# szpajder/dumphfdl

Measured on AMD Instinct MI355X. Metric: wideband I/Q Msamples/s (cf32 ingest -> decoded HFDL PDUs) at fixed channel count, higher is better.
Workload: dtype f32

## Files before the change

### dumphfdl_amd/csrc/frontend.h

```cpp
#pragma once
#include <hip/hip_runtime.h>
#include <deque>
#include <memory>
#include <vector>
#include "../../include/hfdl_gpu.h"
#include "hip_handles.h"
#include "kernels.h"
#include "planner.h"
#include "demod.h"
#include "spectrum.h"
#include "export_ring.h"

namespace hfdl {

int select_device(int device);
long env_long(const char *name, long lo, long hi, long otherwise);
inline int ilog2(int x) { int l = 0; while ((1 << l) < x) l++; return l; }
inline size_t sample_bytes(int fmt) { return fmt == SFMT_CS16 ? 4 : fmt == SFMT_CU8 ? 2 : 8; }
bool is_library_pinned(const void *p, size_t bytes);

struct LabConfig {
	int fold_tile = -1;
	int fold_slices = 0;
	int cu_split = 0;
// ... 62 lines not shown
	PinnedBuf<float> host;
	std::vector<Event> ev;
	std::vector<hfdl_gpu_spectrum_row> info;
	uint64_t open = 0;
	uint64_t open_first = 0;
	uint32_t open_blocks = 0;
	uint64_t oldest() const { const uint64_t kept = (uint64_t)rows - (open_blocks ? 1 : 0); return open > kept ? open - kept : 0; }
	void close()
	{
		info[open % (uint64_t)rows] = hfdl_gpu_spectrum_row{ open, open_first, open_blocks, 0 };
		open++;
		open_blocks = 0;
	}
};

struct SpectrumMonitor {
	int bins = 0;
	uint32_t flags = 0;
	DevBuf acc;
	DevBuf peak;
	PinnedBuf<float> host;
	Event ev;
	hipEvent_t last = nullptr;
	hipEvent_t newest() const { return last ? last : ev.e; }
	uint64_t fresh = 0;
	std::vector<uint64_t> blocks, first;
	std::unique_ptr<SpectrumHistory> hist;
};

struct ChannelExport {
	int nsel = 0, format = 0;
	float scale = 1.f;
	ExportRing ring;
	DevBuf channels;
	DevBuf samples, counts, power, clipped;
	size_t chunk = 1;
	PinnedBuf<char> host;
	std::vector<Event> ev;
	std::vector<uint64_t> last_of;
	hipEvent_t newest = nullptr;
};

}

struct hfdl_gpu_frontend {
	int device = 0;
	hfdl::Stream stream;
	hfdl::Stream stream_b;
	hfdl::Stream stream_d;
	hfdl::Stream stream_c;
	hfdl::Stream stream_f;
	bool cu_partitioned = false;
	bool own_decode_stream() const { return stream_d.owned; }
	bool fft_own_stream() const { return stream_f.owned; }
	static constexpr int MAX_HALF = hfdl::FOLD_MAX_BLOCKS;
	static constexpr int MAX_STAGE = HFDL_GPU_PREFETCH_MAX + 1;
	static_assert(MAX_HALF == hfdl::PLAN_MAX_HALF && MAX_STAGE == hfdl::PLAN_MAX_STAGE && HFDL_GPU_FOLD_BATCH_MAX == MAX_HALF, "include/hfdl_gpu.h, kernels.h and planner.h name the same limits");

	std::deque<hfdl::DevBuf> mem;
	template <typename T> hipError_t alloc(T *&view, size_t count)
	{
		mem.emplace_back();
		const hipError_t e = mem.back().alloc(sizeof(T) * count);
		view = mem.back().as<T>();
		return e;
	}
	hfdl::HostFftPlan fft;
	hfdl::Demod demod;
	int4 *d_rx = nullptr, *d_grp = nullptr;
	float2 *d_hist[2] = { nullptr, nullptr }, *d_work = nullptr, *d_spec = nullptr, *d_taps = nullptr, *d_partial = nullptr;
	float2 *d_tw_m = nullptr;
	int n_stage = 0;
	std::unique_ptr<hfdl::DevBuf> d_stage[MAX_STAGE];
	size_t stage_cap[MAX_STAGE] = {};
	float2 *d_chan_all = nullptr;
	int *d_cnt_all = nullptr;
	hfdl::ChanConst *d_cc = nullptr;
	int2 *d_win = nullptr;
	hfdl::NcoState *d_nco = nullptr;
	hfdl::NcoState *d_nco_snap = nullptr;
	float2 *d_ph = nullptr, *d_ph_cont = nullptr;
	std::unique_ptr<hfdl::SpectrumMonitor> mon;
	std::unique_ptr<hfdl::ChannelExport> exp;

	hfdl::DoneEvent dm[2][MAX_HALF];
	hfdl::DoneEvent chan[2];
	hfdl::DoneEvent fft_done;
	hfdl::DoneEvent spec[2];
	hfdl::Event ev_demod[2];
	hfdl::Event ev_stage_ready[MAX_STAGE];
	hfdl::Event ev_stage_free[MAX_STAGE];
	hfdl::LaunchTimers timers;
	int settle_events();

	uint64_t host_blocks = 0;
	uint64_t host_pushed = 0;
	const void *pf_ptr[MAX_STAGE] = {};
	int pf_fmt[MAX_STAGE] = {};
	hipEvent_t input_event(uint64_t host_block) const
	{
		const uint64_t newest = host_blocks - 1, span = (uint64_t)n_stage - 1;
		return ev_stage_ready[(newest - host_block <= span ? host_block : newest - span) % (uint64_t)n_stage];
	}
	int32_t sample_rate = 0, decimation = 0;
	float tbw = 0;
	hfdl::Plan plan{};
	hfdl::Geometry geo{};
	std::vector<int32_t> freqs;
	int nrx = 1;
	std::vector<int32_t> rx_center;
	std::vector<int32_t> rx_of;
	std::vector<hfdl::RxSpan> rx_span;
	std::vector<int4> rx_host;
	int slot_of(int c) const { return hfdl::receiver_slot(rx_span[(size_t)rx_of[(size_t)c]], c); }
	std::vector<hfdl::ChanConst> cc;
	int batch = 1;
	int fold_nb = 1;
	int half_blocks = 1;
	int half_first = 1, half_target = 1;
	int cur_half = 0, batch_fill = 0;
	int last_slot = 0;
	int last_index = 0;
	float2 *chan_slot(int slot) const { return d_chan_all + (size_t)slot * (size_t)geo.nch * (size_t)geo.outs; }
	int *cnt_slot(int slot) const { return d_cnt_all + (size_t)slot * (size_t)geo.nch; }
	int last_set = 0;
	float2 *spec_slot(int set, int i) const { return d_spec + ((size_t)set * (size_t)half_blocks + (size_t)i) * spec_stride(); }
	size_t spec_stride() const { return (size_t)nrx * (size_t)geo.n; }
	float2 *ph_slot(int set, int i) const { return d_ph + ((size_t)set * (size_t)half_blocks + (size_t)i) * ph_stride(); }
	hfdl::NcoState *snap_slot(int set, int i) const { return d_nco_snap + ((size_t)set * (size_t)half_blocks + (size_t)i) * (size_t)geo.nch; }
	size_t partial_stride() const { return (size_t)geo.nch * (size_t)geo.slices * (size_t)geo.m; }
	size_t ph_stride() const { return (size_t)geo.nch * (size_t)geo.outs; }
	double prune_tol = 0.0;
	int fold_rows_max = 0;
	bool fold_bound = false;
	uint64_t blocks = 0;
	hfdl::FftOutLayout tap_layout;
	int pending_demod_buf = -1;
	int pending_demod_nblk = 0;
	bool frames_wait_on_a = false;
	int demod_buf = -1;
	int prev_demod_buf = -1;
// ... 4 lines not shown
```

### dumphfdl_amd/csrc/frontend_create.cpp

```cpp
#include <atomic>
#include <cmath>
#include <complex>
#include <cstring>
#include <thread>
#include "frontend.h"

using namespace hfdl;

extern "C" int hfdl_gpu_device_count(void)
{
	int n = 0;
	if (hipGetDeviceCount(&n) != hipSuccess) return 0;
	return n;
}

int hfdl::select_device(int device)
{
	int n = 0;
	if (hipGetDeviceCount(&n) != hipSuccess || n <= 0)
		return fail(HFDL_GPU_ENODEV, "no HIP device visible: the HFDL front end has no CPU fallback");
	if (device < 0 || device >= n) return fail(HFDL_GPU_EINVAL, "device %d out of range (%d visible)", device, n);
	HIP_TRY(hipSetDevice(device));
	hipDeviceProp_t prop;
	HIP_TRY(hipGetDeviceProperties(&prop, device));
// ... 126 lines not shown
{
	if (!out || !centerfreqs || !freqs || !nch_per_rx) return fail(HFDL_GPU_EINVAL, "bad arguments: null pointer");
	*out = nullptr;
	if (nrx < 1 || nrx > HFDL_GPU_RECEIVERS_MAX) return fail(HFDL_GPU_EINVAL, "bad arguments: %d receivers (1 .. %d)", nrx, HFDL_GPU_RECEIVERS_MAX);
	for (int r = 0; r < nrx; r++)
		if (nch_per_rx[r] <= 0) return fail(HFDL_GPU_EINVAL, "bad arguments: receiver %d has %d channels", r, nch_per_rx[r]);
	if (sample_rate < 5400) return fail(HFDL_GPU_EINVAL, "sample rate must be >= 5400 (src/main.c:638-641)");
	for (int r = 0, c = 0; r < nrx; r++)
		for (int i = 0; i < nch_per_rx[r]; i++, c++)
			if (std::abs((int64_t)centerfreqs[r] - freqs[c]) >= sample_rate / 2)
				return nrx == 1 ? fail(HFDL_GPU_EINVAL, "channel %d Hz outside +-fs/2 of centre %d", freqs[c], centerfreqs[r])
				                : fail(HFDL_GPU_EINVAL, "channel %d (%d Hz) outside +-fs/2 of the centre %d of its receiver %d", c, freqs[c], centerfreqs[r], r);
	return 0;
}

extern "C" int hfdl_gpu_frontend_create(hfdl_gpu_frontend **out, int device, int32_t sample_rate, int32_t centerfreq,
		const int32_t *freqs, int32_t nch)
{
	if (!out || !freqs || nch <= 0) return fail(HFDL_GPU_EINVAL, "bad arguments");
	return hfdl_gpu_frontend_create_multi(out, device, sample_rate, 1, &centerfreq, freqs, &nch);
}

static int create_streams(hfdl_gpu_frontend *fe, const LabConfig &lab)
{
	CuPartition part = plan_cu_partition((int)fe->freqs.size(), Demod::workgroup_lds(), fe->fold_bound);
	if (!lab.cu_partition || lab.cu_split) part.on = false;
	if (part.on) {
		const hipError_t ea = fe->stream.create_on_cus(part.mask_fold), eb = fe->stream_b.create_on_cus(part.mask_demod);
		if (ea != hipSuccess || eb != hipSuccess) {
			fe->stream.reset(); fe->stream_b.reset();
			(void)hipGetLastError();
			(void)fail(0, "CU-masked streams refused (%s): the demodulators share the fold's CUs", hipGetErrorString(ea != hipSuccess ? ea : eb));
			part.on = false;
		}
	}
	fe->cu_partitioned = part.on;
	if (part.on) {
	} else if (lab.cu_split) {
		uint32_t mask_a[8] = {}, mask_b[8] = {};
		for (int i = 0; i < 256; i++)
			((((i >> 3) + i) % lab.cu_split) == 0 ? mask_b : mask_a)[i >> 5] |= 1u << (i & 31);
		CREATE_TRY(fe->stream.create_on_cus(mask_a));
		CREATE_TRY(fe->stream_b.create_on_cus(mask_b));
	} else {
		CREATE_TRY(fe->stream.create());
		CREATE_TRY(fe->stream_b.create());
	}
	if (lab.decode_stream) CREATE_TRY(fe->stream_d.create());
	else fe->stream_d.alias(fe->stream_b);
	fe->demod.separate_decode = fe->own_decode_stream();
	if (lab.fft_stream < 0 ? part.on : lab.fft_stream != 0) {
		if (part.on) CREATE_TRY(fe->stream_f.create_on_cus(part.mask_fold));
		else CREATE_TRY(fe->stream_f.create());
	} else fe->stream_f.alias(fe->stream);
	CREATE_TRY(fe->stream_c.create());
	return 0;
}

static int create_frontend(hfdl_gpu_frontend *fe, int32_t nrx, const int32_t *nch_per_rx)
{
	const int nch = (int)fe->freqs.size();
	const LabConfig lab = read_lab_config();
	if (!plan_block(fe->plan, fe->tbw, fe->decimation, 0.f)) return fail(HFDL_GPU_EINVAL, "fastddc planning failed");
	const Plan &pl = fe->plan;
	Geometry &g = fe->geo;
	g.n = pl.n; g.m = pl.m; g.pre = pl.pre; g.post = pl.post; g.scrap = pl.scrap; g.post_input_size = pl.post_input_size;
	g.overlap = pl.overlap; g.input_size = pl.input_size; g.outs = (pl.post_input_size + pl.post - 1) / pl.post + 1;
	g.nch = nch;
	g.tap_layout = (pl.m % 16) == 0 && (pl.pre % 8) == 0 ? TAPL_OCTET : TAPL_PLAIN;
	g.nch_pad = plan_receiver_slots(nch_per_rx, nrx, tap_layout_group(g.tap_layout), fe->rx_span);
	for (const RxSpan &r : fe->rx_span) fe->rx_host.push_back(make_int4(r.slot0, r.slots, r.chan0, r.nch));
	g.nrx = nrx;
	g.spec_rx_stride = pl.n;
	g.rx_host = fe->rx_host.data();
	g.tap_chan_stride = pl.m; g.tap_row_stride = (int64_t)g.nch_pad * pl.m;
	g.fold_tile = lab.fold_tile;
	fe->tap_layout.kind = g.tap_layout;
	fe->tap_layout.row_log = ilog2(pl.m); fe->tap_layout.row_stride = g.tap_row_stride;
	fe->prune_tol = g.tap_layout == TAPL_OCTET && nrx == 1 ? env_double("HFDL_GPU_FOLD_PRUNE", 1e-12, 1e-3, 0.0) : 0.0;
	fe->fold_bound = lab.fold_bound < 0 ? nch >= 128 : lab.fold_bound != 0;
	const float resamp_rate = (float)(1800 * 3) / ((float)fe->sample_rate / (float)fe->decimation);
	BatchOverrides ov;
	ov.demod_batch = (int)env_long("HFDL_GPU_DEMOD_BATCH", 1, 8, 0);
	ov.fold_batch = (int)env_long("HFDL_GPU_FOLD_BATCH", 1, hfdl_gpu_frontend::MAX_HALF, 0);
	ov.pruned = fe->prune_tol > 0;
	ov.fold_slices = lab.fold_slices;
	ov.no_ramp = !lab.fold_ramp;
	const BatchPlan bp = plan_batches(nch, nrx, pl.n, pl.input_size, fe->sample_rate, pl.pre, fe->fold_bound,
			[&](int want) { return Demod::fit_batch(g.outs, resamp_rate, want); }, ov);
	g.slices = bp.slices;
	g.rows_per_slice = pl.pre / g.slices;
	if (pl.m > 8192 || pl.m < 16) return fail(HFDL_GPU_ERANGE, "inverse FFT size %d unsupported", pl.m);

	if (int rc = create_streams(fe, lab)) return rc;
	for (int i = 0; i < 2; i++) {
		CREATE_TRY(fe->spec[i].own.create(EV_NO_TIMING));
		CREATE_TRY(fe->chan[i].own.create(EV_NO_TIMING));
		CREATE_TRY(fe->ev_demod[i].create(EV_NO_TIMING));
		for (DoneEvent &d : fe->dm[i]) CREATE_TRY(d.own.create(EV_NO_TIMING));
	}
	CREATE_TRY(fe->fft_done.own.create(EV_NO_TIMING));
	if (int rc = fe->fft.build(pl.n)) return rc;
	const size_t n = (size_t)pl.n;
	const size_t K = (size_t)nrx;
	for (int i = 0; i < 2; i++) {
		CREATE_TRY(fe->alloc(fe->d_hist[i], (size_t)pl.overlap * K));
		CREATE_TRY(hipMemsetAsync(fe->d_hist[i], 0, sizeof(float2) * (size_t)pl.overlap * K, fe->stream));
	}
	CREATE_TRY(fe->alloc(fe->d_work, n * K));
	CREATE_TRY(fe->alloc(fe->d_rx, K));
	CREATE_TRY(hipMemcpy(fe->d_rx, fe->rx_host.data(), sizeof(int4) * K, hipMemcpyHostToDevice));
	g.rx_tab = fe->d_rx;
	if (g.tap_layout == TAPL_OCTET) {
		static_assert(sizeof(FoldGroup) == sizeof(int4), "a FoldGroup entry is what the fold kernels load as an int4");
		const std::vector<FoldGroup> t = fold_group_tables(fe->rx_span, g.nch_pad / 8, FOLD_GROUP_MAX);
		CREATE_TRY(fe->alloc(fe->d_grp, t.size()));
		CREATE_TRY(hipMemcpy(fe->d_grp, t.data(), sizeof(int4) * t.size(), hipMemcpyHostToDevice));
		g.grp_tab = fe->d_grp;
	}
	CREATE_TRY(fe->alloc(fe->d_taps, n * (size_t)g.nch_pad));
	CREATE_TRY(fe->alloc(fe->d_nco, (size_t)nch));
	CREATE_TRY(hipMemsetAsync(fe->d_nco, 0, sizeof(NcoState) * (size_t)nch, fe->stream));
	CREATE_TRY(fe->alloc(fe->d_ph_cont, (size_t)nch));
	CREATE_TRY(fe->alloc(fe->d_cc, (size_t)nch));
	fe->mem.emplace_back();
	if (int rc = upload_twiddles(pl.m, fe->mem.back())) return rc;
	fe->d_tw_m = fe->mem.back().as<float2>();
	if (prepare_ifft_nco(pl.m) != hipSuccess)
		return fail(HFDL_GPU_EHIP, "inverse FFT of %d points: LDS attribute refused: %s", pl.m, hipGetErrorString(hipGetLastError()));
	if (int rc = build_taps(fe)) return rc;
	if (fe->prune_tol > 0 && g.tap_layout == TAPL_OCTET)
		if (int rc = build_fold_windows(fe)) return rc;
	CREATE_TRY(hipMemcpy(fe->d_cc, fe->cc.data(), sizeof(ChanConst) * (size_t)nch, hipMemcpyHostToDevice));
	fe->fold_nb = bp.fold_nb;
	if (int rc = fe->demod.init(nch, g.outs, resamp_rate, fe->freqs.data(), fe->stream, bp.batch_want)) return rc;
	fe->batch = fe->demod.batch;
	fe->half_blocks = bp.half_blocks;
	fe->half_first = fe->half_target = bp.half_first;
	fe->n_stage = bp.n_stage;
	for (int i = 0; i < fe->n_stage; i++) {
		CREATE_TRY(fe->ev_stage_ready[i].create(EV_NO_TIMING));
		CREATE_TRY(fe->ev_stage_free[i].create(EV_NO_TIMING));
	}
	const size_t hb = (size_t)fe->half_blocks;
	CREATE_TRY(fe->alloc(fe->d_spec, fe->spec_stride() * 2 * hb));
	CREATE_TRY(fe->alloc(fe->d_partial, fe->partial_stride() * hb));
	CREATE_TRY(fe->alloc(fe->d_ph, fe->ph_stride() * 2 * hb));
	CREATE_TRY(fe->alloc(fe->d_nco_snap, (size_t)nch * 2 * hb));
	CREATE_TRY(fe->alloc(fe->d_chan_all, 2 * hb * (size_t)nch * g.outs));
	CREATE_TRY(fe->alloc(fe->d_cnt_all, 2 * hb * (size_t)nch));
	CREATE_TRY(hipMemsetAsync(fe->d_cnt_all, 0, sizeof(int) * 2 * hb * (size_t)nch, fe->stream));
	CREATE_TRY(hipStreamSynchronize(fe->stream));
	return 0;
}
// ... 31 lines not shown
```

### dumphfdl_amd/csrc/frontend_query.cpp

```cpp
#include <algorithm>
#include <cstdarg>
#include <cstdio>
#include <cstring>
#include <mutex>
#include "frontend.h"

using namespace hfdl;

static thread_local char g_err[512] = "";

int hfdl::fail(int code, const char *fmt, ...)
{
	va_list ap;
	va_start(ap, fmt);
	vsnprintf(g_err, sizeof(g_err), fmt, ap);
	va_end(ap);
	return code;
}

int hfdl::fail_hip(hipError_t e, bool alloc, const char *expr, const char *file, int line)
{
	return fail(alloc && e == hipErrorOutOfMemory ? HFDL_GPU_ENOMEM : HFDL_GPU_EHIP, "%s: %s (%s:%d)", expr, hipGetErrorString(e), file, line);
}

// ... 33 lines not shown
	memset(g, 0, sizeof(*g));
	fill_block_geometry(p, g);
	g->decimation = decimation;
	g->transition_bw = transition_bw;
	return 0;
}

extern "C" int hfdl_gpu_frontend_channel_receiver(const hfdl_gpu_frontend *fe, int32_t channel, int32_t *rx, int32_t *centerfreq)
{
	if (!fe || !rx || !centerfreq) return fail(HFDL_GPU_EINVAL, "null argument");
	if (channel < 0 || channel >= fe->geo.nch) return fail(HFDL_GPU_EINVAL, "channel %d out of range (%d channels)", channel, fe->geo.nch);
	*rx = fe->rx_of[(size_t)channel];
	*centerfreq = fe->rx_center[(size_t)*rx];
	return 0;
}


static std::mutex g_pinned_lock;
static std::vector<std::pair<const char *, size_t>> g_pinned;

bool hfdl::is_library_pinned(const void *p, size_t bytes)
{
	std::lock_guard<std::mutex> lk(g_pinned_lock);
	for (auto &r : g_pinned)
		if ((const char *)p >= r.first && (const char *)p + bytes <= r.first + r.second) return true;
	return false;
}

extern "C" int hfdl_gpu_host_alloc(void **ptr, size_t bytes)
{
	if (!ptr || !bytes) return fail(HFDL_GPU_EINVAL, "bad arguments");
	HIP_TRY(hipHostMalloc(ptr, bytes, hipHostMallocDefault));
	std::lock_guard<std::mutex> lk(g_pinned_lock);
	g_pinned.emplace_back((const char *)*ptr, bytes);
	return 0;
}

extern "C" void hfdl_gpu_host_free(void *ptr)
{
	if (!ptr) return;
	{
		std::lock_guard<std::mutex> lk(g_pinned_lock);
		for (size_t i = 0; i < g_pinned.size(); i++)
			if (g_pinned[i].first == (const char *)ptr) { g_pinned.erase(g_pinned.begin() + (long)i); break; }
	}
	(void)hipHostFree(ptr);
}


extern "C" int hfdl_gpu_frontend_input_done(hfdl_gpu_frontend *fe)
{
	if (!fe) return fail(HFDL_GPU_EINVAL, "null argument");
	HIP_TRY(hipSetDevice(fe->device));
	HIP_TRY(hipStreamSynchronize(fe->stream_c));
	return 0;
}

static int check_host_block(const hfdl_gpu_frontend *fe, uint64_t host_block)
{
	if (!fe) return fail(HFDL_GPU_EINVAL, "null argument");
	if (host_block >= fe->host_blocks) return fail(HFDL_GPU_EINVAL, "host block %llu has not been pushed (%llu so far)", (unsigned long long)host_block, (unsigned long long)fe->host_blocks);
	HIP_TRY(hipSetDevice(fe->device));
	return 0;
}

extern "C" int hfdl_gpu_frontend_input_done_upto(hfdl_gpu_frontend *fe, uint64_t host_block)
{
	if (int rc = check_host_block(fe, host_block)) return rc;
	HIP_TRY(hipEventSynchronize(fe->input_event(host_block)));
	return 0;
}

extern "C" int hfdl_gpu_frontend_input_copied(hfdl_gpu_frontend *fe, uint64_t host_block)
{
	if (int rc = check_host_block(fe, host_block)) return rc;
	const hipError_t e = hipEventQuery(fe->input_event(host_block));
	if (e == hipSuccess) return 1;
	if (e == hipErrorNotReady) { (void)hipGetLastError(); return 0; }
	return fail(HFDL_GPU_EHIP, "hipEventQuery: %s", hipGetErrorString(e));
}


static int sync_to_read(hfdl_gpu_frontend *fe, bool args_ok = true)
{
	if (!fe || !args_ok) return fail(HFDL_GPU_EINVAL, "null argument");
	return hfdl_gpu_frontend_sync(fe);
}

extern "C" int hfdl_gpu_frontend_reset_timers(hfdl_gpu_frontend *fe, int enable)
{
	if (int rc = sync_to_read(fe)) return rc;
	return fe->timers.reset(enable != 0);
}

static int stage_totals(hfdl_gpu_frontend *fe, Stage s, double *ms, int64_t *launches, int64_t *blocks)
{
	if (int rc = sync_to_read(fe)) return rc;
	const LaunchTimers::Totals &t = fe->timers.stage[s];
	if (ms) *ms = t.ms;
	if (launches) *launches = t.launches;
	if (blocks) *blocks = t.blocks;
	return 0;
}

extern "C" int hfdl_gpu_frontend_fold_time_ms(hfdl_gpu_frontend *fe, double *total_ms, int64_t *launches) { return stage_totals(fe, ST_FOLD, total_ms, launches, nullptr); }

extern "C" int hfdl_gpu_frontend_fold_blocks(hfdl_gpu_frontend *fe, int64_t *blocks)
// ... 362 lines not shown
```

### dumphfdl_amd/csrc/hfdl_gpu.cpp

```cpp
#include <algorithm>
#include "frontend.h"

using namespace hfdl;


int LaunchTimers::arm(Stage s, int blocks, hipEvent_t &start, hipEvent_t &stop)
{
	if (!on) return 0;
	Timed t;
	if (!pool.empty()) {
		t = std::move(pool.back());
		pool.pop_back();
	} else {
		HIP_TRY(t.start.create(EV_TIMING));
		HIP_TRY(t.stop.create(EV_TIMING));
	}
	t.blocks = blocks;
	start = t.start;
	stop = t.stop;
	stage[s].pending.push_back(std::move(t));
	return 0;
}

int LaunchTimers::drain()
{
	for (int s = 0; s < ST_N; s++) {
		for (Timed &t : stage[s].pending) {
			float ms = 0;
			HIP_TRY(hipEventElapsedTime(&ms, t.start, t.stop));
			stage[s].ms += ms;
			stage[s].launches++;
			stage[s].blocks += t.blocks;
			if (s == ST_FOLD) {
				fold_last_blocks = t.blocks;
				if (t.blocks >= 1 && t.blocks <= FOLD_MAX_BLOCKS) { fold_shapes[t.blocks]++; fold_shape_ms[t.blocks] += ms; }
				if (!first_fold) {
					first_fold = std::move(t.start);
					HIP_TRY(t.start.create(EV_TIMING));
				} else {
					HIP_TRY(hipEventElapsedTime(&ms, first_fold, t.start));
					span_ms = ms;
				}
			}
			pool.push_back(std::move(t));
		}
		stage[s].pending.clear();
	}
	return 0;
}

int LaunchTimers::reset(bool enable)
{
	on = enable;
	for (Totals &t : stage) { t.ms = 0; t.launches = 0; t.blocks = 0; }
	for (auto &c : fold_shapes) c = 0;
	for (auto &c : fold_shape_ms) c = 0;
	first_fold = Event();
	span_ms = 0;
	fold_last_blocks = 0;
	while (enable && pool.size() < 1280) {
		Timed t;
		HIP_TRY(t.start.create(EV_TIMING));
		HIP_TRY(t.stop.create(EV_TIMING));
		pool.push_back(std::move(t));
	}
	return 0;
}

int hfdl_gpu_frontend::settle_events()
{
	if (int rc = timers.drain()) return rc;
	for (auto &half : dm) for (DoneEvent &d : half) d.settle();
	for (DoneEvent *d : { &chan[0], &chan[1], &fft_done, &spec[0], &spec[1] }) d->settle();
	return 0;
}


extern "C" void *hfdl_gpu_frontend_stream(hfdl_gpu_frontend *fe) { return fe ? (void *)fe->stream_f.s : nullptr; }

static int check_block(const hfdl_gpu_frontend *fe, size_t nsamples, int fmt)
{
	if (fmt != SFMT_CF32 && fmt != SFMT_CS16 && fmt != SFMT_CU8) return fail(HFDL_GPU_EINVAL, "unknown sample format %d", fmt);
	if (nsamples != (size_t)fe->plan.input_size)
		return fail(HFDL_GPU_EINVAL, "a block is exactly %d samples (got %zu)", fe->plan.input_size, nsamples);
	return 0;
}

static int queue_input_copy(hfdl_gpu_frontend *fe, const void *const *iq, size_t nsamples, int fmt, int *sb_out)
{
	if (fe->host_blocks - fe->host_pushed >= (uint64_t)fe->n_stage)
		return fail(HFDL_GPU_ERANGE, "%d uploads are queued ahead of their blocks: push the oldest first", fe->n_stage);
	const uint64_t j = fe->host_blocks;
	const int sb = (int)(j % (uint64_t)fe->n_stage);
	const size_t need = nsamples * (size_t)fe->nrx;
	if (fe->stage_cap[sb] < need) {
		HIP_TRY(hipStreamSynchronize(fe->stream_c));
		HIP_TRY(hipStreamSynchronize(fe->stream_f));
		fe->stage_cap[sb] = 0;
		fe->d_stage[sb] = std::make_unique<DevBuf>();
		HIP_TRY(fe->d_stage[sb]->alloc(sizeof(float2) * need));
		fe->stage_cap[sb] = need;
	}
	HIP_TRY(hipStreamWaitEvent(fe->stream_c, fe->ev_stage_free[sb], 0));
	const size_t bytes = sample_bytes(fmt) * nsamples;
	bool pinned = true;
	for (int r = 0; r < fe->nrx; r++) {
		HIP_TRY(hipMemcpyAsync(fe->d_stage[sb]->as<char>() + (size_t)r * bytes, iq[r], bytes, hipMemcpyHostToDevice, fe->stream_c));
		pinned = pinned && is_library_pinned(iq[r], bytes);
	}
	HIP_TRY(hipEventRecord(fe->ev_stage_ready[sb], fe->stream_c));
	fe->host_blocks = j + 1;
	if (!pinned) HIP_TRY(hipStreamSynchronize(fe->stream_c));
	*sb_out = sb;
	return 0;
}

static int stage_input(hfdl_gpu_frontend *fe, const void *const *iq, size_t nsamples, int fmt, int on_device, FftInputs &in, int *stage_idx)
{
	*stage_idx = -1;
	if (!fe || !iq) return fail(HFDL_GPU_EINVAL, "null argument");
	for (int r = 0; r < fe->nrx; r++) if (!iq[r]) return fail(HFDL_GPU_EINVAL, "null argument: the block of receiver %d", r);
	if (int rc = check_block(fe, nsamples, fmt)) return rc;
	HIP_TRY(hipSetDevice(fe->device));
	const bool queued = fe->host_pushed < fe->host_blocks;
	if (on_device) {
		if (queued) return fail(HFDL_GPU_EINVAL, "a prefetched block is pending: push it or call hfdl_gpu_frontend_prefetch_cancel()");
		for (int r = 0; r < fe->nrx; r++) in.fresh[r] = iq[r];
		return 0;
	}
	int sb;
	if (queued) {
		sb = (int)(fe->host_pushed % (uint64_t)fe->n_stage);
		if (fe->pf_ptr[sb] != iq[0] || fe->pf_fmt[sb] != fmt) return fail(HFDL_GPU_EINVAL, "the block pushed after a prefetch must be the (oldest) prefetched one");
	} else {
		int rc = queue_input_copy(fe, iq, nsamples, fmt, &sb);
		if (rc) return rc;
	}
	fe->host_pushed++;
	HIP_TRY(hipStreamWaitEvent(fe->stream_f, fe->ev_stage_ready[sb], 0));
	for (int r = 0; r < fe->nrx; r++) in.fresh[r] = fe->d_stage[sb]->as<const char>() + (size_t)r * sample_bytes(fmt) * nsamples;
	*stage_idx = sb;
	return 0;
}

static int single_receiver_only(const hfdl_gpu_frontend *fe, const char *what)
{
	if (fe && fe->nrx > 1)
		return fail(HFDL_GPU_EINVAL, "%s: this front end has %d receivers -- push a block of every receiver with hfdl_gpu_frontend_push_blocks_raw()", what, fe->nrx);
	return 0;
}

extern "C" int hfdl_gpu_frontend_prefetch_block_raw(hfdl_gpu_frontend *fe, const void *raw, size_t nsamples, int sample_format)
{
	if (!fe || !raw) return fail(HFDL_GPU_EINVAL, "null argument");
	if (int rc = single_receiver_only(fe, "hfdl_gpu_frontend_prefetch_block_raw")) return rc;
	if (int rc = check_block(fe, nsamples, sample_format)) return rc;
	if (fe->host_blocks - fe->host_pushed >= (uint64_t)(fe->n_stage - 1))
		return fail(HFDL_GPU_ERANGE, "%d blocks are prefetched already (geometry.prefetch_depth): push the oldest first", fe->n_stage - 1);
	if (!is_library_pinned(raw, sample_bytes(sample_format) * nsamples)) return fail(HFDL_GPU_EINVAL, "only buffers from hfdl_gpu_host_alloc() can be prefetched");
	HIP_TRY(hipSetDevice(fe->device));
	int sb = -1;
	const void *one[1] = { raw };
	int rc = queue_input_copy(fe, one, nsamples, sample_format, &sb);
	if (rc) return rc;
	fe->pf_ptr[sb] = raw; fe->pf_fmt[sb] = sample_format;
	return 0;
}

extern "C" int hfdl_gpu_frontend_prefetch_cancel(hfdl_gpu_frontend *fe)
{
	if (!fe) return fail(HFDL_GPU_EINVAL, "null argument");
	if (int rc = single_receiver_only(fe, "hfdl_gpu_frontend_prefetch_cancel")) return rc;
	if (fe->host_pushed == fe->host_blocks) return 0;
	HIP_TRY(hipSetDevice(fe->device));
	HIP_TRY(hipStreamSynchronize(fe->stream_c));
	fe->host_pushed = fe->host_blocks;
	return 0;
}


static int launch_demod(hfdl_gpu_frontend *fe, int buf, int nblk, bool after_fft)
{
	HIP_TRY(hipStreamWaitEvent(fe->stream_b, after_fft ? fe->fft_done.event() : fe->chan[buf].event(), 0));
	const int launches = (nblk + fe->batch - 1) / fe->batch;
	for (int j0 = 0, l = 0; j0 < nblk; j0 += fe->batch, l++) {
		const int take = std::min(fe->batch, nblk - j0);
		DoneEvent &done = fe->dm[buf][launches - 1 - l];
		hipEvent_t t_start = nullptr;
		int rc = fe->timers.arm(ST_DEMOD, take, done, t_start);
		if (rc) return rc;
		const int slot = buf * fe->half_blocks + j0;
		rc = fe->demod.enqueue_demod(fe->chan_slot(slot), fe->cnt_slot(slot), take, fe->stream_b, done.event(), l == 0 && fe->frames_wait_on_a, t_start);
		if (rc) return rc;
		if (fe->own_decode_stream()) HIP_TRY(hipStreamWaitEvent(fe->stream_d, done.event(), 0));
		hipEvent_t k5_start = nullptr, k5_stop = nullptr;
		if ((rc = fe->timers.arm(ST_DECODE, take, k5_start, k5_stop))) return rc;
		if ((rc = fe->demod.enqueue_decode(buf, fe->stream_d, k5_start, k5_stop))) return rc;
	}
	fe->frames_wait_on_a = false;
	HIP_TRY(hipEventRecord(fe->ev_demod[buf], fe->stream_d));
	return 0;
}

static int flush_pending_demod(hfdl_gpu_frontend *fe, bool after_fft)
{
	if (fe->pending_demod_buf < 0) return 0;
	const int buf = fe->pending_demod_buf, nblk = fe->pending_demod_nblk;
	fe->pending_demod_buf = -1;
	return launch_demod(fe, buf, nblk, after_fft);
}

static int enqueue_fft(hfdl_gpu_frontend *fe, FftInputs &in, int fmt, int stage_idx)
{
	const Geometry &g = fe->geo;
	const int i = fe->batch_fill, set = fe->cur_half;
	const bool pend = !fe->fft_own_stream() && fe->pending_demod_buf >= 0 && i + 1 == fe->half_target;
	if (fe->fft_own_stream() && i == 0) HIP_TRY(hipStreamWaitEvent(fe->stream_f, fe->chan[set].event(), 0));
	NcoJob job;
	job.cc = fe->d_cc; job.chain = fe->d_nco; job.snap = fe->snap_slot(set, i);
	job.ph = fe->ph_slot(set, i); job.cont = fe->d_ph_cont;
	job.nch = g.nch; job.outs = g.outs; job.post_input_size = g.post_input_size; job.post = g.post;
	hipEvent_t fft_start = nullptr, fft_done = nullptr;
	if (fe->fft_own_stream()) fft_done = fe->spec[set].signal();
	else if (int rc = pend ? fe->timers.arm(ST_FFT, 1, fe->fft_done, fft_start) : fe->timers.arm(ST_FFT, 1, fft_start, fft_done)) return rc;
	if (pend) fft_done = fe->fft_done.event();
	in.nrx = fe->nrx; in.hist_stride = g.overlap; in.out_stride = g.n;
	launch_fft_forward(fe->fft.p, fe->d_hist[fe->blocks & 1], in, fmt, g.overlap, fe->d_hist[(fe->blocks + 1) & 1], fe->d_work, fe->spec_slot(set, i), true, fe->stream_f,
			FftOutLayout(), fft_done, job,
			stage_idx >= 0 ? fe->ev_stage_free[stage_idx].e : nullptr,
			fft_start);
	if (SpectrumMonitor *mon = fe->mon.get()) {
		SpecmonJob m;
		m.spec = fe->spec_slot(set, i); m.rx_stride = g.n; m.n = g.n; m.bins = mon->bins; m.nrx = fe->nrx; m.flags = mon->flags;
		m.scale = (float)(1.0 / ((double)g.n * (double)g.n * ((mon->flags & SPECMON_HANN) ? 0.375 : 1.0)));
		m.fresh = mon->fresh; m.acc = mon->acc.as<float2>(); m.peak = mon->peak.as<float>();
		SpectrumHistory *h = mon->hist.get();
		hipEvent_t done = mon->ev;
		if (h) {
			const size_t slot = (size_t)(h->open % (uint64_t)h->rows), set = (size_t)fe->nrx * (size_t)mon->bins;
			m.row_acc = h->acc.as<float2>() + slot * set;
			if (mon->flags & SPECMON_MAXHOLD) m.row_peak = h->peak.as<float>() + slot * set;
			m.row_fresh = h->open_blocks == 0;
			done = h->ev[slot];
		}
		launch_spectrum_monitor(m, fe->stream_f, done);
		mon->last = done;
		for (int r = 0; r < fe->nrx; r++) {
			if ((mon->fresh >> r) & 1) { mon->blocks[(size_t)r] = 0; mon->first[(size_t)r] = fe->blocks; }
			mon->blocks[(size_t)r]++;
		}
		if (h) {
			if (h->open_blocks++ == 0) h->open_first = fe->blocks;
			if (h->interval > 0 && h->open_blocks == (uint32_t)h->interval) h->close();
		}
		mon->fresh = 0;
	}
	if (pend) {
		int rc = flush_pending_demod(fe, true);
		if (rc) return rc;
	}
	HIP_TRY(hipGetLastError());
	fe->blocks++;
	fe->batch_fill++;
	return 0;
}

static int close_half(hfdl_gpu_frontend *fe, bool launch_now, bool with_demod = true)
{
	const int nblk = fe->batch_fill;
	if (nblk == 0) return 0;
	const Geometry &g = fe->geo;
	const int half = fe->cur_half;
	if (fe->fft_own_stream()) HIP_TRY(hipStreamWaitEvent(fe->stream, fe->spec[half].event(), 0));
	for (int done = 0, take = 0; done < nblk; done += take) {
		take = fold_launch_blocks(g, nblk - done, fe->fold_nb);
		hipEvent_t start = nullptr, stop = nullptr;
		if (int rc = fe->timers.arm(ST_FOLD, take, start, stop)) return rc;
		if (launch_fold(g, fe->d_taps, fe->spec_slot(half, done), fe->spec_stride(), fe->d_partial + (size_t)done * fe->partial_stride(), fe->partial_stride(),
				take, fe->stream, start, stop) < 0)
			return fail(HFDL_GPU_EINVAL, "no fold launch of %d blocks on this geometry", take);
	}
	if (fe->dm[half][0].pending()) HIP_TRY(hipStreamWaitEvent(fe->stream, fe->dm[half][0].event(), 0));
	if (with_demod && fe->own_decode_stream() && !fe->fold_bound) {
		hipEvent_t e = fe->demod.frames_free_event();
		if (e) HIP_TRY(hipStreamWaitEvent(fe->stream, e, 0));
		fe->frames_wait_on_a = true;
	}
	const int slot0 = half * fe->half_blocks;
	hipEvent_t ifft_start = nullptr;
	if (int rc = fe->timers.arm(ST_IFFT, nblk, fe->chan[half], ifft_start)) return rc;
	launch_ifft_nco(g, fe->d_partial, fe->partial_stride(), fe->d_cc, fe->snap_slot(half, 0), fe->ph_slot(half, 0), fe->ph_stride(), fe->d_tw_m,
			fe->chan_slot(slot0), fe->cnt_slot(slot0), nblk, fe->stream, fe->chan[half].event(), ifft_start);
	if (ChannelExport *x = fe->exp.get()) {
		const uint32_t skip = x->ring.skip_of_half(fe->blocks - (uint64_t)nblk, (uint32_t)nblk);
		if (skip < (uint32_t)nblk) {
			ExportJob e;
			e.chan = fe->chan_slot(slot0 + (int)skip); e.cnt = fe->cnt_slot(slot0 + (int)skip); e.channels = x->channels.as<int32_t>();
			e.nch = g.nch; e.outs = g.outs; e.P = g.outs - 1; e.nsel = x->nsel; e.nblk = nblk - (int)skip; e.format = x->format; e.scale = x->scale;
			e.slot0 = x->ring.slot(fe->blocks - (uint64_t)e.nblk); e.R = x->ring.R;
			e.samples = x->samples.p; e.counts = x->counts.as<int32_t>(); e.power = x->power.as<float>(); e.clipped = x->clipped.as<uint32_t>();
			x->newest = x->ev[x->ring.push_launch(x->last_of.data(), fe->blocks - 1)];
			launch_export_pack(e, fe->stream, x->newest);
		}
	}
	HIP_TRY(hipGetLastError());
	fe->last_slot = slot0 + nblk - 1;
	fe->last_index = nblk - 1;
	fe->last_set = half;
	fe->cur_half ^= 1;
	fe->batch_fill = 0;
	if (!with_demod) return 0;
	fe->prev_demod_buf = fe->demod_buf;
	fe->demod_buf = half;
	if (launch_now || fe->fft_own_stream()) return launch_demod(fe, half, nblk, false);
	fe->pending_demod_buf = half;
	fe->pending_demod_nblk = nblk;
	return 0;
}

extern "C" int hfdl_gpu_frontend_channelize_block(hfdl_gpu_frontend *fe, const float *iq, size_t nsamples, int on_device)
{
	FftInputs in;
	int sidx = -1;
	int rc = single_receiver_only(fe, "hfdl_gpu_frontend_channelize_block");
	if (rc) return rc;
	const void *one[1] = { iq };
	if ((rc = stage_input(fe, one, nsamples, SFMT_CF32, on_device, in, &sidx))) return rc;
	if ((rc = flush_pending_demod(fe, false))) return rc;
	if ((rc = close_half(fe, true))) return rc;
	if ((rc = enqueue_fft(fe, in, SFMT_CF32, sidx))) return rc;
	return close_half(fe, false, false);
}

extern "C" int hfdl_gpu_frontend_push_baseband(hfdl_gpu_frontend *fe, const float *chan_out, const int32_t *counts)
{
	if (!fe || !chan_out || !counts) return fail(HFDL_GPU_EINVAL, "null argument");
	const Geometry &g = fe->geo;
	for (int c = 0; c < g.nch; c++)
		if (counts[c] < 0 || counts[c] > g.outs) return fail(HFDL_GPU_ERANGE, "channel %d: %d samples, a block holds at most %d", c, counts[c], g.outs);
	int rc = hfdl_gpu_frontend_sync(fe);
	if (rc) return rc;
	const int half = fe->cur_half, slot0 = half * fe->half_blocks;
	HIP_TRY(hipMemcpy(fe->chan_slot(slot0), chan_out, sizeof(float2) * (size_t)g.nch * (size_t)g.outs, hipMemcpyHostToDevice));
	HIP_TRY(hipMemcpy(fe->cnt_slot(slot0), counts, sizeof(int32_t) * (size_t)g.nch, hipMemcpyHostToDevice));
	fe->last_slot = slot0;
	fe->last_index = 0;
	fe->cur_half ^= 1;
	fe->prev_demod_buf = fe->demod_buf;
	fe->demod_buf = half;
	return launch_demod(fe, half, 1, false);
}

static int push_any(hfdl_gpu_frontend *fe, const void *const *raw, size_t nsamples, int fmt, int on_device)
{
	FftInputs in;
	int sidx = -1;
	int rc = stage_input(fe, raw, nsamples, fmt, on_device, in, &sidx);
	if (rc) return rc;
	if ((rc = enqueue_fft(fe, in, fmt, sidx))) return rc;
	if (fe->batch_fill < fe->half_target) return 0;
	rc = close_half(fe, !fe->fold_bound);
	fe->half_target = fe->half_blocks;
	return rc;
}

extern "C" int hfdl_gpu_frontend_push_block(hfdl_gpu_frontend *fe, const float *iq, size_t nsamples, int on_device)
{
	if (int rc = single_receiver_only(fe, "hfdl_gpu_frontend_push_block")) return rc;
	const void *one[1] = { iq };
	return push_any(fe, one, nsamples, SFMT_CF32, on_device);
}

extern "C" int hfdl_gpu_frontend_push_block_raw(hfdl_gpu_frontend *fe, const void *raw, size_t nsamples, int sample_format, int on_device)
{
	if (int rc = single_receiver_only(fe, "hfdl_gpu_frontend_push_block_raw")) return rc;
	const void *one[1] = { raw };
	return push_any(fe, one, nsamples, sample_format, on_device);
}

extern "C" int hfdl_gpu_frontend_push_blocks_raw(hfdl_gpu_frontend *fe, const void *const *raw, size_t nsamples, int sample_format, int on_device)
{
	if (!fe || !raw) return fail(HFDL_GPU_EINVAL, "null argument");
	return push_any(fe, raw, nsamples, sample_format, on_device);
}


extern "C" int hfdl_gpu_frontend_sync(hfdl_gpu_frontend *fe)
{
	if (!fe) return fail(HFDL_GPU_EINVAL, "null argument");
	HIP_TRY(hipSetDevice(fe->device));
	{ int rc = flush_pending_demod(fe, false); if (rc) return rc; }
	{ int rc = close_half(fe, true); if (rc) return rc; }
	fe->half_target = fe->half_first;
	for (const Stream *s : { &fe->stream_c, &fe->stream_f, &fe->stream, &fe->stream_b, &fe->stream_d }) HIP_TRY(s->sync());
	HIP_TRY(hipGetLastError());
	return fe->settle_events();
}

static int check_poll_args(const hfdl_gpu_frontend *fe, const hfdl_gpu_pdu *out, int32_t max, const int32_t *n)
{
	if (!fe || !n) return fail(HFDL_GPU_EINVAL, "null argument");
	if (!out && max > 0) return fail(HFDL_GPU_EINVAL, "null PDU buffer with max = %d", max);
	return 0;
}

extern "C" int hfdl_gpu_frontend_poll_pdus(hfdl_gpu_frontend *fe, hfdl_gpu_pdu *out, int32_t max, int32_t *n)
{
	int rc = check_poll_args(fe, out, max, n);
	if (rc || (rc = hfdl_gpu_frontend_sync(fe))) return rc;
	return fe->demod.collect(out, max, n, fe->stream_d);
}

extern "C" int hfdl_gpu_frontend_poll_pdus_ready(hfdl_gpu_frontend *fe, hfdl_gpu_pdu *out, int32_t max, int32_t *n, int32_t max_in_flight)
{
	if (max_in_flight <= 0) return hfdl_gpu_frontend_poll_pdus(fe, out, max, n);
	if (int rc = check_poll_args(fe, out, max, n)) return rc;
	*n = 0;
	const int buf = fe->prev_demod_buf;
	if (buf < 0) return 0;
	HIP_TRY(hipSetDevice(fe->device));
	const hipEvent_t ev = fe->dm[buf][0].event();
	if (max_in_flight >= 2) {
		const hipError_t q = hipEventQuery(ev);
		if (q == hipErrorNotReady) { (void)hipGetLastError(); return 0; }
		if (q != hipSuccess) return fail(HFDL_GPU_EHIP, "hipEventQuery: %s", hipGetErrorString(q));
	} else {
		HIP_TRY(hipEventSynchronize(ev));
	}
	const bool decoded = hipEventQuery(fe->ev_demod[buf]) == hipSuccess;
	if (!decoded) (void)hipGetLastError();
	return fe->demod.collect_snapshot(decoded ? buf : buf ^ 1, out, max, n, fe->stream_d);
}
```

### dumphfdl_amd/csrc/planner.h

```cpp
#pragma once
#include <algorithm>
#include <cmath>
#include <cstdint>
#include <vector>
#include <complex>

namespace hfdl {

struct Plan {
	int32_t pre, post, taps_min_length, taps_length, overlap, n, m, input_size, post_input_size, scrap, v;
	int32_t startbin, offsetbin;
	float pre_shift, post_shift, sindelta, cosdelta, rate;
};

inline int32_t pow2_above(int32_t x)
{
	int32_t p = 1;
	for (int i = 0; i < 31; i++, p <<= 1) if (x < p) return p;
	return -1;
}

inline int32_t fft_decimation_rate(int32_t fs, int32_t target)
{
	return pow2_above((int32_t)std::floor((float)fs / (float)target)) / 2;
// ... 119 lines not shown
	int fold_batch = 0;
	bool pruned = false;
	int fold_slices = 0;
	bool no_ramp = false;
};

struct BatchPlan {
	int slices;
	int fold_nb;
	int batch_want;
	int half_blocks;
	int half_first;
	int n_stage;
};

constexpr int PLAN_MAX_HALF = 32;
constexpr int PLAN_MAX_STAGE = 18;

template <typename Fit>
inline BatchPlan plan_batches(int nch, int nrx, int n, int input_size, int sample_rate, int pre, bool fold_bound, Fit demod_fit, const BatchOverrides &ov)
{
	BatchPlan b{};
	b.slices = pick_slices(nch, pre);
	if (ov.fold_slices > 0 && (ov.fold_slices & (ov.fold_slices - 1)) == 0 && pre % ov.fold_slices == 0 && pre / ov.fold_slices >= 16) b.slices = ov.fold_slices;
	if (ov.pruned) b.slices = 1;

	b.fold_nb = ov.fold_batch ? ov.fold_batch : (fold_bound ? 32 : 8);

	int want = (int)std::floor(1.0 / ((double)input_size / (double)sample_rate));
	want = std::max(1, std::min(8, want));
	if (fold_bound) want = std::min(want, 3);
	if (ov.demod_batch) want = ov.demod_batch;
	want = demod_fit(want);
	if (nrx > 1) {
		const int64_t cap = std::max<int64_t>(1, ((int64_t)32 << 23) / ((int64_t)nrx * (int64_t)n));
		if (cap < std::max(b.fold_nb, want)) {
			b.fold_nb = (int)std::min<int64_t>(b.fold_nb, cap);
			want = std::min(want, b.fold_nb);
		}
	}
	if (!ov.demod_batch && want < b.fold_nb) {
		const int launches = (b.fold_nb + want - 1) / want;
		want = (b.fold_nb + launches - 1) / launches;
	}
	b.batch_want = want;
	const int batch = demod_fit(want);
	b.half_blocks = std::min(PLAN_MAX_HALF, ((std::max(b.fold_nb, batch) + b.fold_nb - 1) / b.fold_nb) * b.fold_nb);
	b.half_first = (fold_bound && b.half_blocks > 16 && !ov.no_ramp) ? 16 : b.half_blocks;
	b.n_stage = std::min(b.half_blocks + 2, PLAN_MAX_STAGE);
	return b;
}


constexpr int PLAN_CUS = 256, PLAN_XCDS = 8, PLAN_CU_LDS = 160 * 1024;
constexpr int PLAN_DEMOD_WG_PER_CU = 4;
struct CuPartition {
	bool on = false;
	int wg_per_cu = 0, demod_cus = 0;
	uint32_t mask_fold[PLAN_CUS / 32] = {}, mask_demod[PLAN_CUS / 32] = {};
};
inline CuPartition plan_cu_partition(int nch, size_t demod_lds, bool fold_bound)
{
	CuPartition p;
	if (!fold_bound || nch < 1 || demod_lds == 0 || demod_lds > (size_t)PLAN_CU_LDS) return p;
	p.wg_per_cu = std::min<int>(PLAN_DEMOD_WG_PER_CU, (int)((size_t)PLAN_CU_LDS / demod_lds));
	const int cus = (nch + p.wg_per_cu - 1) / p.wg_per_cu, per_xcd = (cus + PLAN_XCDS - 1) / PLAN_XCDS;
	if (per_xcd > PLAN_CUS / PLAN_XCDS / 2) return p;
	for (int m = 0; m < PLAN_XCDS; m++)
		for (int q = 0; q < per_xcd; q++) {
			const int i = (4 * m + (q & 3)) * 8 + ((m + (q & 3) + 2 * (q >> 2)) & 7);
			p.mask_demod[i >> 5] |= 1u << (i & 31);
		}
	for (int w = 0; w < PLAN_CUS / 32; w++) p.mask_fold[w] = ~p.mask_demod[w];
	p.demod_cus = per_xcd * PLAN_XCDS;
	p.on = true;
	return p;
}


struct RowWindow { int32_t first, count; };
inline std::vector<RowWindow> fold_row_windows(const std::vector<float> &en, int p, int npad, int nch, double tol, int *rows_max)
{
	std::vector<std::vector<char>> keep((size_t)npad, std::vector<char>((size_t)p, 0));
	for (int c = 0; c < nch; c++) {
		double tot = 0;
		int peak = 0;
		for (int r = 0; r < p; r++) { tot += en[(size_t)r * npad + c]; if (en[(size_t)r * npad + c] > en[(size_t)peak * npad + c]) peak = r; }
		auto e_at = [&](int r) { return (double)en[(size_t)((r % p + p) % p) * npad + c]; };
		int lo = peak, hi = peak;
		double left = tot - e_at(peak);
		while (hi - lo + 1 < p && left > tol * tol * tot) {
			if (e_at(lo - 1) > e_at(hi + 1)) left -= e_at(--lo); else left -= e_at(++hi);
		}
		for (int r = lo; r <= hi; r++) keep[(size_t)c][(size_t)((r % p + p) % p)] = 1;
	}
	auto hull = [&](int c0, int c1) {
		const int nq = p / 4;
		std::vector<char> any((size_t)nq, 0);
		int kept = 0;
		for (int c = c0; c < c1; c++) for (int r = 0; r < p; r++) if (keep[(size_t)c][(size_t)r] && !any[(size_t)(r >> 2)]) { any[(size_t)(r >> 2)] = 1; kept++; }
		if (kept == 0) return RowWindow{ 0, 2 };
		int best_len = 0, best_end = 0;
		for (int q = 0; q < nq; q++) {
			if (any[(size_t)q] || !any[(size_t)((q + nq - 1) % nq)]) continue;
			int len = 0;
			while (len < nq && !any[(size_t)((q + len) % nq)]) len++;
// ... 14 lines not shown
```

Baseline: 19830.

## Choose FFT stream per push from input residency with explicit ordering plan

Adds an FftOrder planner that decides, for each pushed block, whether the forward FFT runs serially on the main stream or beside it on a separate stream. By default the choice follows where the input lives: device-resident input goes beside, host input stays serial. The planner inserts the needed cross-stream waits, flushes and demod hold-backs when the side changes. Several full-stream synchronizations are replaced by waits on the specific stage-ready events, which cuts host stalls on the copy stream but adds ordering logic that could introduce races or extra waits.

```diff
diff --git a/dumphfdl_amd/csrc/frontend.h b/dumphfdl_amd/csrc/frontend.h
--- a/dumphfdl_amd/csrc/frontend.h
+++ b/dumphfdl_amd/csrc/frontend.h
@@ -138,7 +138,10 @@
 	hfdl::Stream stream_f;
 	bool cu_partitioned = false;
 	bool own_decode_stream() const { return stream_d.owned; }
-	bool fft_own_stream() const { return stream_f.owned; }
+	hfdl::FftRule fft_rule = hfdl::FFT_RULE_INPUT;
+	hfdl::FftOrder order;
+	int side_of(bool on_device) const { return hfdl::fft_side(fft_rule, on_device); }
+	hipStream_t fft_stream(int side) const { return side == hfdl::FFT_SERIAL ? stream.s : stream_f.owned ? stream_f.s : stream_c.s; }
 	static constexpr int MAX_HALF = hfdl::FOLD_MAX_BLOCKS;
 	static constexpr int MAX_STAGE = HFDL_GPU_PREFETCH_MAX + 1;
 	static_assert(MAX_HALF == hfdl::PLAN_MAX_HALF && MAX_STAGE == hfdl::PLAN_MAX_STAGE && HFDL_GPU_FOLD_BATCH_MAX == MAX_HALF, "include/hfdl_gpu.h, kernels.h and planner.h name the same limits");
@@ -173,6 +176,7 @@
 	hfdl::DoneEvent chan[2];
 	hfdl::DoneEvent fft_done;
 	hfdl::DoneEvent spec[2];
+	hfdl::Event ev_switch;
 	hfdl::Event ev_demod[2];
 	hfdl::Event ev_stage_ready[MAX_STAGE];
 	hfdl::Event ev_stage_free[MAX_STAGE];
diff --git a/dumphfdl_amd/csrc/frontend_create.cpp b/dumphfdl_amd/csrc/frontend_create.cpp
--- a/dumphfdl_amd/csrc/frontend_create.cpp
+++ b/dumphfdl_amd/csrc/frontend_create.cpp
@@ -202,7 +202,8 @@
 	if (lab.fft_stream < 0 ? part.on : lab.fft_stream != 0) {
 		if (part.on) CREATE_TRY(fe->stream_f.create_on_cus(part.mask_fold));
 		else CREATE_TRY(fe->stream_f.create());
-	} else fe->stream_f.alias(fe->stream);
+		fe->fft_rule = FFT_RULE_OWN;
+	} else if (lab.fft_stream == 0) fe->fft_rule = FFT_RULE_SERIAL;
 	CREATE_TRY(fe->stream_c.create());
 	return 0;
 }
@@ -250,6 +251,7 @@
 		for (DoneEvent &d : fe->dm[i]) CREATE_TRY(d.own.create(EV_NO_TIMING));
 	}
 	CREATE_TRY(fe->fft_done.own.create(EV_NO_TIMING));
+	CREATE_TRY(fe->ev_switch.create(EV_NO_TIMING));
 	if (int rc = fe->fft.build(pl.n)) return rc;
 	const size_t n = (size_t)pl.n;
 	const size_t K = (size_t)nrx;
diff --git a/dumphfdl_amd/csrc/frontend_query.cpp b/dumphfdl_amd/csrc/frontend_query.cpp
--- a/dumphfdl_amd/csrc/frontend_query.cpp
+++ b/dumphfdl_amd/csrc/frontend_query.cpp
@@ -109,7 +109,7 @@
 {
 	if (!fe) return fail(HFDL_GPU_EINVAL, "null argument");
 	HIP_TRY(hipSetDevice(fe->device));
-	HIP_TRY(hipStreamSynchronize(fe->stream_c));
+	if (fe->host_blocks) HIP_TRY(hipEventSynchronize(fe->input_event(fe->host_blocks - 1)));
 	return 0;
 }
 
diff --git a/dumphfdl_amd/csrc/hfdl_gpu.cpp b/dumphfdl_amd/csrc/hfdl_gpu.cpp
--- a/dumphfdl_amd/csrc/hfdl_gpu.cpp
+++ b/dumphfdl_amd/csrc/hfdl_gpu.cpp
@@ -76,7 +76,7 @@
 }
 
 
-extern "C" void *hfdl_gpu_frontend_stream(hfdl_gpu_frontend *fe) { return fe ? (void *)fe->stream_f.s : nullptr; }
+extern "C" void *hfdl_gpu_frontend_stream(hfdl_gpu_frontend *fe) { return fe ? (void *)fe->fft_stream(fe->side_of(true)) : nullptr; }
 
 static int check_block(const hfdl_gpu_frontend *fe, size_t nsamples, int fmt)
 {
@@ -95,7 +95,7 @@
 	const size_t need = nsamples * (size_t)fe->nrx;
 	if (fe->stage_cap[sb] < need) {
 		HIP_TRY(hipStreamSynchronize(fe->stream_c));
-		HIP_TRY(hipStreamSynchronize(fe->stream_f));
+		HIP_TRY(hipStreamSynchronize(fe->fft_stream(fe->side_of(false))));
 		fe->stage_cap[sb] = 0;
 		fe->d_stage[sb] = std::make_unique<DevBuf>();
 		HIP_TRY(fe->d_stage[sb]->alloc(sizeof(float2) * need));
@@ -110,7 +110,7 @@
 	}
 	HIP_TRY(hipEventRecord(fe->ev_stage_ready[sb], fe->stream_c));
 	fe->host_blocks = j + 1;
-	if (!pinned) HIP_TRY(hipStreamSynchronize(fe->stream_c));
+	if (!pinned) HIP_TRY(hipEventSynchronize(fe->ev_stage_ready[sb]));
 	*sb_out = sb;
 	return 0;
 }
@@ -137,7 +137,7 @@
 		if (rc) return rc;
 	}
 	fe->host_pushed++;
-	HIP_TRY(hipStreamWaitEvent(fe->stream_f, fe->ev_stage_ready[sb], 0));
+	HIP_TRY(hipStreamWaitEvent(fe->fft_stream(fe->side_of(false)), fe->ev_stage_ready[sb], 0));
 	for (int r = 0; r < fe->nrx; r++) in.fresh[r] = fe->d_stage[sb]->as<const char>() + (size_t)r * sample_bytes(fmt) * nsamples;
 	*stage_idx = sb;
 	return 0;
@@ -173,7 +173,7 @@
 	if (int rc = single_receiver_only(fe, "hfdl_gpu_frontend_prefetch_cancel")) return rc;
 	if (fe->host_pushed == fe->host_blocks) return 0;
 	HIP_TRY(hipSetDevice(fe->device));
-	HIP_TRY(hipStreamSynchronize(fe->stream_c));
+	HIP_TRY(hipEventSynchronize(fe->input_event(fe->host_blocks - 1)));
 	fe->host_pushed = fe->host_blocks;
 	return 0;
 }
@@ -210,22 +210,32 @@
 	return launch_demod(fe, buf, nblk, after_fft);
 }
 
-static int enqueue_fft(hfdl_gpu_frontend *fe, FftInputs &in, int fmt, int stage_idx)
+static int enqueue_fft(hfdl_gpu_frontend *fe, FftInputs &in, int fmt, int stage_idx, int on_device)
 {
 	const Geometry &g = fe->geo;
 	const int i = fe->batch_fill, set = fe->cur_half;
-	const bool pend = !fe->fft_own_stream() && fe->pending_demod_buf >= 0 && i + 1 == fe->half_target;
-	if (fe->fft_own_stream() && i == 0) HIP_TRY(hipStreamWaitEvent(fe->stream_f, fe->chan[set].event(), 0));
+	const FftPushPlan plan = fe->order.push(fe->side_of(on_device != 0), i, fe->half_target, fe->pending_demod_buf >= 0);
+	const hipStream_t st = fe->fft_stream(plan.side);
+	if (plan.flush_before)
+		if (int rc = flush_pending_demod(fe, false)) return rc;
+	if (plan.wait_switch) {
+		HIP_TRY(hipEventRecord(fe->ev_switch, fe->fft_stream(plan.side ^ 1)));
+		HIP_TRY(hipStreamWaitEvent(st, fe->ev_switch, 0));
+	}
+	if (plan.wait_set_free && fe->chan[set].pending()) HIP_TRY(hipStreamWaitEvent(st, fe->chan[set].event(), 0));
+	if (plan.wait_first_fold) HIP_TRY(hipStreamWaitEvent(st, fe->chan[set ^ 1].event(), 0));
 	NcoJob job;
 	job.cc = fe->d_cc; job.chain = fe->d_nco; job.snap = fe->snap_slot(set, i);
 	job.ph = fe->ph_slot(set, i); job.cont = fe->d_ph_cont;
 	job.nch = g.nch; job.outs = g.outs; job.post_input_size = g.post_input_size; job.post = g.post;
 	hipEvent_t fft_start = nullptr, fft_done = nullptr;
-	if (fe->fft_own_stream()) fft_done = fe->spec[set].signal();
-	else if (int rc = pend ? fe->timers.arm(ST_FFT, 1, fe->fft_done, fft_start) : fe->timers.arm(ST_FFT, 1, fft_start, fft_done)) return rc;
-	if (pend) fft_done = fe->fft_done.event();
+	if (plan.side == FFT_BESIDE || plan.hold_after) {
+		DoneEvent &done = plan.side == FFT_BESIDE ? fe->spec[set] : fe->fft_done;
+		if (int rc = fe->timers.arm(ST_FFT, 1, done, fft_start)) return rc;
+		fft_done = done.event();
+	} else if (int rc = fe->timers.arm(ST_FFT, 1, fft_start, fft_done)) return rc;
 	in.nrx = fe->nrx; in.hist_stride = g.overlap; in.out_stride = g.n;
-	launch_fft_forward(fe->fft.p, fe->d_hist[fe->blocks & 1], in, fmt, g.overlap, fe->d_hist[(fe->blocks + 1) & 1], fe->d_work, fe->spec_slot(set, i), true, fe->stream_f,
+	launch_fft_forward(fe->fft.p, fe->d_hist[fe->blocks & 1], in, fmt, g.overlap, fe->d_hist[(fe->blocks + 1) & 1], fe->d_work, fe->spec_slot(set, i), true, st,
 			FftOutLayout(), fft_done, job,
 			stage_idx >= 0 ? fe->ev_stage_free[stage_idx].e : nullptr,
 			fft_start);
@@ -243,7 +253,7 @@
 			m.row_fresh = h->open_blocks == 0;
 			done = h->ev[slot];
 		}
-		launch_spectrum_monitor(m, fe->stream_f, done);
+		launch_spectrum_monitor(m, st, done);
 		mon->last = done;
 		for (int r = 0; r < fe->nrx; r++) {
 			if ((mon->fresh >> r) & 1) { mon->blocks[(size_t)r] = 0; mon->first[(size_t)r] = fe->blocks; }
@@ -255,7 +265,7 @@
 		}
 		mon->fresh = 0;
 	}
-	if (pend) {
+	if (plan.hold_after) {
 		int rc = flush_pending_demod(fe, true);
 		if (rc) return rc;
 	}
@@ -271,7 +281,8 @@
 	if (nblk == 0) return 0;
 	const Geometry &g = fe->geo;
 	const int half = fe->cur_half;
-	if (fe->fft_own_stream()) HIP_TRY(hipStreamWaitEvent(fe->stream, fe->spec[half].event(), 0));
+	const HalfClosePlan plan = fe->order.close(launch_now);
+	if (plan.wait_input) HIP_TRY(hipStreamWaitEvent(fe->stream, fe->spec[half].event(), 0));
 	for (int done = 0, take = 0; done < nblk; done += take) {
 		take = fold_launch_blocks(g, nblk - done, fe->fold_nb);
 		hipEvent_t start = nullptr, stop = nullptr;
@@ -312,7 +323,7 @@
 	if (!with_demod) return 0;
 	fe->prev_demod_buf = fe->demod_buf;
 	fe->demod_buf = half;
-	if (launch_now || fe->fft_own_stream()) return launch_demod(fe, half, nblk, false);
+	if (!plan.hold_back) return launch_demod(fe, half, nblk, false);
 	fe->pending_demod_buf = half;
 	fe->pending_demod_nblk = nblk;
 	return 0;
@@ -328,7 +339,7 @@
 	if ((rc = stage_input(fe, one, nsamples, SFMT_CF32, on_device, in, &sidx))) return rc;
 	if ((rc = flush_pending_demod(fe, false))) return rc;
 	if ((rc = close_half(fe, true))) return rc;
-	if ((rc = enqueue_fft(fe, in, SFMT_CF32, sidx))) return rc;
+	if ((rc = enqueue_fft(fe, in, SFMT_CF32, sidx, on_device))) return rc;
 	return close_half(fe, false, false);
 }
 
@@ -357,7 +368,7 @@
 	int sidx = -1;
 	int rc = stage_input(fe, raw, nsamples, fmt, on_device, in, &sidx);
 	if (rc) return rc;
-	if ((rc = enqueue_fft(fe, in, fmt, sidx))) return rc;
+	if ((rc = enqueue_fft(fe, in, fmt, sidx, on_device))) return rc;
 	if (fe->batch_fill < fe->half_target) return 0;
 	rc = close_half(fe, !fe->fold_bound);
 	fe->half_target = fe->half_blocks;
@@ -393,6 +404,7 @@
 	{ int rc = close_half(fe, true); if (rc) return rc; }
 	fe->half_target = fe->half_first;
 	for (const Stream *s : { &fe->stream_c, &fe->stream_f, &fe->stream, &fe->stream_b, &fe->stream_d }) HIP_TRY(s->sync());
+	fe->order.drained();
 	HIP_TRY(hipGetLastError());
 	return fe->settle_events();
 }
diff --git a/dumphfdl_amd/csrc/planner.h b/dumphfdl_amd/csrc/planner.h
--- a/dumphfdl_amd/csrc/planner.h
+++ b/dumphfdl_amd/csrc/planner.h
@@ -195,6 +195,40 @@
 }
 
 
+enum FftSide { FFT_SERIAL = 0, FFT_BESIDE = 1 };
+enum FftRule { FFT_RULE_INPUT, FFT_RULE_SERIAL, FFT_RULE_OWN };
+inline int fft_side(FftRule rule, bool on_device) { return rule == FFT_RULE_INPUT ? (on_device ? FFT_BESIDE : FFT_SERIAL) : rule == FFT_RULE_OWN ? FFT_BESIDE : FFT_SERIAL; }
+
+struct FftPushPlan { int side; bool wait_switch, wait_set_free, wait_first_fold, flush_before, hold_after; };
+struct HalfClosePlan { bool wait_input, hold_back; };
+struct FftOrder {
+	int prev_side = -1;
+	bool half_beside = false;
+	int halves = 0;
+	FftPushPlan push(int side, int fill, int target, bool held_back)
+	{
+		FftPushPlan p{};
+		p.side = side;
+		p.wait_switch = prev_side >= 0 && prev_side != side;
+		p.wait_set_free = side == FFT_BESIDE && fill == 0;
+		p.wait_first_fold = side == FFT_BESIDE && fill == 0 && halves == 1;
+		p.flush_before = side == FFT_BESIDE && held_back;
+		p.hold_after = side == FFT_SERIAL && held_back && fill + 1 == target;
+		prev_side = side;
+		half_beside = half_beside || side == FFT_BESIDE;
+		return p;
+	}
+	HalfClosePlan close(bool launch_now)
+	{
+		const HalfClosePlan c{ half_beside, !launch_now && prev_side == FFT_SERIAL };
+		half_beside = false;
+		halves++;
+		return c;
+	}
+	void drained() { prev_side = -1; halves = 0; }
+};
+
+
 constexpr int PLAN_CUS = 256, PLAN_XCDS = 8, PLAN_CU_LDS = 160 * 1024;
 constexpr int PLAN_DEMOD_WG_PER_CU = 4;
 struct CuPartition {
```

New measurement: 21300 (median of 6 runs). 7.4% higher.
